# MakiseChris666/MVXNet-Makise

Measured on AMD Instinct MI355X. Metric: KITTI frames/sec (voxelize+VFE+fusion+3Dconv fwd+bwd), higher is better.
Workload: dtype f32 (bf16x6: three bf16 pieces = the f32 operand exactly, six MFMAs per product, f32 accumulate); 1 GPU; S2 ring frames (64-beam model, KITTI-like occupancy), 120000 raw pts -> 20000 pts after crop, grid 10x352x400, T=35, 4 frames/GPU/step: crop+cropToSight+lidar2Img, voxelize, fusion sampling+MLP, VFE, reindex+CML fwd+bwd, all-reduce, AdamW; convmath=bf16x6; mode=hot, frames_per_gpu=4, parallelism=dp1

## Files before the change

### mvxnet-makise_amd/csrc/activity.hip

```cpp
#include "common.h"

namespace {

constexpr int ATH = 8, ATW = 16;

__global__ void activity_sites(const void *__restrict__ src, int src_is_index, int Din, int Dout, int H, int W, int sd,
                               int pd, int mark_border, unsigned char *__restrict__ dst, int n_frames) {
    const size_t n = (size_t)n_frames * Dout * H * W;
    for (size_t e = blockIdx.x * (size_t)blockDim.x + threadIdx.x; e < n; e += (size_t)gridDim.x * blockDim.x) {
        const int x = (int)(e % W), y = (int)((e / W) % H), d = (int)(e / ((size_t)W * H));
        int on = mark_border && (y == 0 || y == H - 1 || x == 0 || x == W - 1);
        for (int kd = 0; kd < 3 && !on; ++kd) {
            const int ds = mvx_src_plane(d, Din, Dout, sd, pd, kd);
            if (ds < 0) continue;
            for (int a = -1; a <= 1 && !on; ++a) {
                const int yy = y + a;
                if (yy < 0 || yy >= H) continue;
                for (int b = -1; b <= 1; ++b) {
                    const int xx = x + b;
                    if (xx < 0 || xx >= W) continue;
                    const size_t s = ((size_t)ds * H + yy) * W + xx;
                    on |= src_is_index ? (((const int *)src)[s] >= 0) : (((const unsigned char *)src)[s] != 0);
                }
            }
        }
        dst[e] = (unsigned char)on;
    }
}


__global__ __launch_bounds__(256) void activity_sites4(const void *__restrict__ src, int src_is_index, int Din, int Dout, int H,
                                                       int W, int sd, int pd, int mark_border, unsigned char *__restrict__ dst,
                                                       int n_frames) {
    const int W4 = W >> 2;
    const size_t n = (size_t)n_frames * Dout * H * W4;
    for (size_t e = blockIdx.x * (size_t)blockDim.x + threadIdx.x; e < n; e += (size_t)gridDim.x * blockDim.x) {
        const int x = (int)(e % W4) * 4, y = (int)((e / W4) % H), d = (int)(e / ((size_t)W4 * H));
        unsigned on = 0u;
        if (mark_border) {
            if (y == 0 || y == H - 1) on = 15u;
            if (x == 0) on |= 1u;
            if (x + 4 == W) on |= 8u;
        }
        for (int kd = 0; kd < 3 && on != 15u; ++kd) {
            const int ds = mvx_src_plane(d, Din, Dout, sd, pd, kd);
            if (ds < 0) continue;
            for (int a = -1; a <= 1 && on != 15u; ++a) {
                const int yy = y + a;
                if (yy < 0 || yy >= H) continue;
                const size_t s = ((size_t)ds * H + yy) * W + x;
                unsigned m;
                if (src_is_index) {
                    const int *row = (const int *)src + s;
                    const int4 v = *(const int4 *)row;
                    m = (v.x >= 0 ? 2u : 0u) | (v.y >= 0 ? 4u : 0u) | (v.z >= 0 ? 8u : 0u) | (v.w >= 0 ? 16u : 0u);
                    if (x > 0 && row[-1] >= 0) m |= 1u;
                    if (x + 4 < W && row[4] >= 0) m |= 32u;
                } else {
                    const unsigned char *row = (const unsigned char *)src + s;
                    const unsigned v = *(const unsigned *)row;
                    m = ((v & 0xffu) ? 2u : 0u) | ((v & 0xff00u) ? 4u : 0u) | ((v & 0xff0000u) ? 8u : 0u) | ((v & 0xff000000u) ? 16u : 0u);
                    if (x > 0 && row[-1]) m |= 1u;
                    if (x + 4 < W && row[4]) m |= 32u;
                }
                on |= (m | (m >> 1) | (m >> 2)) & 15u;
            }
        }
        *(unsigned *)(dst + e * 4) = ((on & 1u) ? 1u : 0u) | ((on & 2u) ? 0x100u : 0u) | ((on & 4u) ? 0x10000u : 0u) | ((on & 8u) ? 0x1000000u : 0u);
    }
}

__global__ __launch_bounds__(256) void activity_halo_flags(const unsigned char *__restrict__ mask, int D, int H, int W,
                                                           int *__restrict__ flags, int *__restrict__ tile_flags) {
    const int tiles_x = (W + ATW - 1) / ATW;
    const int tx0 = (blockIdx.x % tiles_x) * ATW - 1, ty0 = (blockIdx.x / tiles_x) * ATH - 1;
    const int d = blockIdx.y;
    int on = 0, inner = 0;
    if (threadIdx.x < (ATH + 2) * (ATW + 2)) {
        const int hy = threadIdx.x / (ATW + 2), hx = threadIdx.x % (ATW + 2);
        const int y = ty0 + hy, x = tx0 + hx;
        if (y >= 0 && y < H && x >= 0 && x < W) on = mask[((size_t)d * H + y) * W + x];
        inner = on && hy >= 1 && hy <= ATH && hx >= 1 && hx <= ATW;
    }
    on = __syncthreads_or(on);
    inner = __syncthreads_or(inner);
    if (threadIdx.x == 0) {
        if (flags) flags[(size_t)d * gridDim.x + blockIdx.x] = on ? 1 : 0;
        if (tile_flags) tile_flags[(size_t)d * gridDim.x + blockIdx.x] = inner ? 1 : 0;
    }
}

__global__ void tile_dilate_flags(const int *__restrict__ in, const int *__restrict__ self, int Din, int Dout, int tiles_y,
                                  int tiles_x, int sd, int pd, int *__restrict__ out, int n_frames) {
    const int e = blockIdx.x * blockDim.x + threadIdx.x;
    const int nt = tiles_y * tiles_x;
    if (e >= n_frames * Dout * nt) return;
    const int d = e / nt, t = e - d * nt, ty = t / tiles_x, tx = t - ty * tiles_x;
    int on = self ? self[e] : 0;
    for (int kd = 0; kd < 3 && !on; ++kd) {
        const int ds = mvx_src_plane(d, Din, Dout, sd, pd, kd);
        if (ds < 0) continue;
        for (int a = -1; a <= 1 && !on; ++a)
            for (int b = -1; b <= 1; ++b) {
                const int yy = ty + a, xx = tx + b;
                if (yy >= 0 && yy < tiles_y && xx >= 0 && xx < tiles_x) on |= in[(size_t)ds * nt + yy * tiles_x + xx];
            }
    }
    out[e] = on ? 1 : 0;
}

__global__ __launch_bounds__(64) void conv_background(const float *__restrict__ w, const float *__restrict__ c_in, int Din,
                                                      int Dout, int Cin, int Cout, int sd, int pd,
                                                      float *__restrict__ bg_pre, float *__restrict__ bg_tap,
                                                      float *__restrict__ bg_cls) {
    const int n = blockIdx.x, d = blockIdx.y;
    double s = 0.0;
    double cls[9];
#pragma unroll
    for (int q = 0; q < 9; ++q) cls[q] = 0.0;
    for (int kd = 0; kd < 3; ++kd) {
        const int ds = mvx_src_plane(d, Din, Dout, sd, pd, kd);
        double sk = 0.0;
        if (ds >= 0)
            for (int e = threadIdx.x; e < Cin * 9; e += 64) {
                const int c = e / 9, k = e - c * 9, a = k / 3, b = k - a * 3;
                const double t = (double)w[(((size_t)n * Cin + c) * 3 + kd) * 9 + k] * (double)c_in[(size_t)ds * Cin + c];
                sk += t;
                if (bg_cls) {
#pragma unroll
                    for (int q = 0; q < 9; ++q) {
                        const int ry = q / 3, rx = q - ry * 3;
                        const bool inside = !(ry == 0 && a == 0) && !(ry == 2 && a == 2) && !(rx == 0 && b == 0) && !(rx == 2 && b == 2);
                        if (inside) cls[q] += t;
                    }
                }
            }
        s += sk;
        if (bg_tap) {
            sk = wave_sum_f64(sk);
            if (threadIdx.x == 0) bg_tap[((size_t)d * 3 + kd) * Cout + n] = (float)sk;
        }
    }
    s = wave_sum_f64(s);
    if (threadIdx.x == 0) bg_pre[(size_t)d * Cout + n] = (float)s;
    if (bg_cls) {
#pragma unroll
        for (int q = 0; q < 9; ++q) {
            const double v = wave_sum_f64(cls[q]);
            if (threadIdx.x == 0) bg_cls[((size_t)d * 9 + q) * Cout + n] = (float)v;
        }
    }
}

__global__ void bn_background(const float *__restrict__ bg_pre, const float *__restrict__ bias, const float *__restrict__ mi,
                              int D, int C, int relu, float *__restrict__ y_bg, float *__restrict__ c_out, int n_frames) {
    const int e = blockIdx.x * blockDim.x + threadIdx.x;
    if (e >= n_frames * D * C) return;
    const int c = e % C;
    mi += (size_t)(e / (D * C)) * 2 * C;
    float v = (bg_pre ? bg_pre[e] : 0.f) + (bias ? bias[c] : 0.f);
    if (relu) v = fmaxf(v, 0.f);
    if (y_bg) y_bg[e] = v;
    c_out[e] = (v - mi[c]) * mi[C + c];
}

__global__ __launch_bounds__(256) void bn_apply_tiles(const float *__restrict__ y, const float *__restrict__ mi,
                                                      const float *__restrict__ c_bg, const int *__restrict__ tile_flags,
                                                      float *__restrict__ out, int D, int H, int W, int C, int ntiles,
                                                      const int *__restrict__ read_flags) {
    const int tiles_x = (W + ATW - 1) / ATW;
    const int t = blockIdx.x, d = blockIdx.y, frame = d / D;
    if (read_flags && !read_flags[(size_t)d * ntiles + t] && !tile_flags[(size_t)d * ntiles + t]) return;
    const int c4n = C >> 2, ct = threadIdx.x % c4n, st = threadIdx.x / c4n, spb = 256 / c4n;
    const int ty0 = (t / tiles_x) * ATH, tx0 = (t % tiles_x) * ATW;
    const bool on = tile_flags[(size_t)d * ntiles + t] != 0;
    const float4 cb = *(const float4 *)(c_bg + (size_t)d * C + ct * 4);
    const float *fmi = mi + (size_t)frame * 2 * C;
    const float4 m = *(const float4 *)(fmi + ct * 4), iv = *(const float4 *)(fmi + C + ct * 4);
    for (int sidx = st; sidx < ATH * ATW; sidx += spb) {
        const int gy = ty0 + sidx / ATW, gx = tx0 + sidx % ATW;
        if (gy >= H || gx >= W) continue;
        const size_t off = (((size_t)d * H + gy) * W + gx) * C + ct * 4;
        float4 o = cb;
        if (on) {
            const float4 v = *(const float4 *)(y + off);
            o = make_float4((v.x - m.x) * iv.x, (v.y - m.y) * iv.y, (v.z - m.z) * iv.z, (v.w - m.w) * iv.w);
        }
        *(float4 *)(out + off) = o;
    }
}

__global__ void tile_read_flags(const int *__restrict__ hflag, int Din, int Dout, int ty_n, int tx_n, int sd, int pd,
                                int *__restrict__ read, int n_frames) {
    const int ntiles = ty_n * tx_n;
    const long long e = blockIdx.x * (long long)blockDim.x + threadIdx.x;
    if (e >= (long long)n_frames * Din * ntiles) return;
    const int p = (int)(e / ntiles), t = (int)(e - (long long)p * ntiles);
    const int ty = t / tx_n, tx = t - ty * tx_n;
    int r = 0;
    for (int kd = 0; kd < 3 && !r; ++kd) {
        const int d = mvx_dst_plane(p, Din, Dout, sd, pd, kd);
        if (d < 0) continue;
        for (int y = max(ty - 1, 0); y <= min(ty + 1, ty_n - 1) && !r; ++y)
            for (int x = max(tx - 1, 0); x <= min(tx + 1, tx_n - 1) && !r; ++x) {
                const int y0 = y & ~1, y1 = min(y0 + 1, ty_n - 1);
                const bool border = x == 0 || x == tx_n - 1 || y0 == 0 || y1 == ty_n - 1;
                int c = border ? 1 : 0;
                for (int k2 = 0; k2 < 3 && !c; ++k2) {
                    const int ds = mvx_src_plane(d, Din, Dout, sd, pd, k2);
                    if (ds >= 0) c = hflag[(size_t)ds * ntiles + y0 * tx_n + x] | hflag[(size_t)ds * ntiles + y1 * tx_n + x];
                }
                r |= c;
            }
    }
    read[e] = r;
}

__global__ __launch_bounds__(256) void bn_apply_tiles_bev(const float *__restrict__ y, const float *__restrict__ mi,
                                                          const float *__restrict__ c_bg, const int *__restrict__ tile_flags,
                                                          float *__restrict__ bev, int D, int H, int W, int C, int ntiles) {
    __shared__ float s_t[ATH * ATW][64 + 1];
    const int tiles_x = (W + ATW - 1) / ATW;
    const int t = blockIdx.x, d = blockIdx.y, frame = d / D, dd = d - frame * D;
    const int c4n = C >> 2, ct = threadIdx.x % c4n, st = threadIdx.x / c4n, spb = 256 / c4n;
    const int ty0 = (t / tiles_x) * ATH, tx0 = (t % tiles_x) * ATW;
    const bool on = tile_flags[(size_t)d * ntiles + t] != 0;
    const float4 cb = *(const float4 *)(c_bg + (size_t)d * C + ct * 4);
    const float *fmi = mi + (size_t)frame * 2 * C;
    const float4 m = *(const float4 *)(fmi + ct * 4), iv = *(const float4 *)(fmi + C + ct * 4);
    for (int sidx = st; sidx < ATH * ATW; sidx += spb) {
        const int gy = ty0 + sidx / ATW, gx = tx0 + sidx % ATW;
        float4 o = cb;
        if (on && gy < H && gx < W) {
            const float4 v = *(const float4 *)(y + (((size_t)d * H + gy) * W + gx) * C + ct * 4);
            o = make_float4((v.x - m.x) * iv.x, (v.y - m.y) * iv.y, (v.z - m.z) * iv.z, (v.w - m.w) * iv.w);
        }
        s_t[sidx][ct * 4 + 0] = o.x; s_t[sidx][ct * 4 + 1] = o.y; s_t[sidx][ct * 4 + 2] = o.z; s_t[sidx][ct * 4 + 3] = o.w;
    }
    __syncthreads();
    float *fb = bev + (size_t)frame * C * D * H * W;
    for (int e = threadIdx.x; e < C * ATH * (ATW / 4); e += 256) {
        const int g4 = e % (ATW / 4), c = (e / (ATW / 4)) % C, r = e / (C * (ATW / 4));
        const int gy = ty0 + r, gx = tx0 + g4 * 4;
        if (gy >= H || gx >= W) continue;
        const int s0 = r * ATW + g4 * 4;
        float *dst = fb + (((size_t)c * D + dd) * H + gy) * W + gx;
        if (gx + 3 < W && (W & 3) == 0) {
            *(float4 *)dst = make_float4(s_t[s0][c], s_t[s0 + 1][c], s_t[s0 + 2][c], s_t[s0 + 3][c]);
        } else {
            for (int j = 0; j < 4 && gx + j < W; ++j) dst[j] = s_t[s0 + j][c];
        }
    }
}

constexpr int BREP = 8;

constexpr int BNB_MAX_PLANES = 16 * MVX_MAX_FRAMES;
__global__ __launch_bounds__(1024) void bnb_tile_list(const int *__restrict__ tile_flags, int D, int H, int W, int ntiles,
                                                      int *__restrict__ list, int *__restrict__ n_act,
                                                      int *__restrict__ n_inact, unsigned *__restrict__ amax_slot) {
    __shared__ int smem[17];
    if (amax_slot && threadIdx.x == 0) *amax_slot = 0u;
    __shared__ int s_inact[BNB_MAX_PLANES];
    const int tiles_x = (W + ATW - 1) / ATW;
    if (threadIdx.x < BNB_MAX_PLANES) s_inact[threadIdx.x] = 0;
    __syncthreads();
    const int total = D * ntiles;
    int base = 0;
    for (int s0 = 0; s0 < total; s0 += 1024 * 64) {
        const int left = total - s0;
        const int per = left >= 1024 * 64 ? 64 : (left + 1023) / 1024;
        const int b0 = s0 + (int)threadIdx.x * per;
        unsigned long long bits = 0ull;
#pragma unroll 8
        for (int k = 0; k < per; ++k) {
            const int e = b0 + k;
            if (e < total) bits |= (unsigned long long)(tile_flags[e] != 0) << k;
        }
        for (int k = 0; k < per; ++k) {
            const int e = b0 + k;
            if (e < total && !((bits >> k) & 1ull)) {
                const int d = e / ntiles, t = e - d * ntiles;
                const int ty0 = (t / tiles_x) * ATH, tx0 = (t % tiles_x) * ATW;
                atomicAdd(&s_inact[d], min(ATH, H - ty0) * min(ATW, W - tx0));
            }
        }
        int tot;
        int pos = base + block_excl_scan_i32(__popcll(bits), smem, &tot);
        while (bits) {
            const int k = __ffsll((long long)bits) - 1;
            bits &= bits - 1;
            list[pos++] = b0 + k;
        }
        base += tot;
    }
    __syncthreads();
    if (threadIdx.x == 0) *n_act = base;
    if (threadIdx.x < D) n_inact[threadIdx.x] = s_inact[threadIdx.x];
}

template <int MODE>
__global__ __launch_bounds__(256) void bnb_tiles(const float *__restrict__ dyh, const float *__restrict__ y,
                                                 const float *__restrict__ mi, const float *__restrict__ c_bg,
                                                 const float *__restrict__ ab, const int *__restrict__ list,
                                                 const int *__restrict__ n_act, int D, int H, int W, int C, int ntiles,
                                                 float *__restrict__ dz, double *__restrict__ sums_all,
                                                 unsigned *__restrict__ amax_slot) {
    __shared__ float red[2][256][4];
    float mx = 0.f;
    const int tiles_x = (W + ATW - 1) / ATW;
    const int c4n = C >> 2, ct = threadIdx.x % c4n, st = threadIdx.x / c4n, spb = 256 / c4n;
    const int nact = *n_act;
    const int per = (nact + (int)gridDim.x - 1) / (int)gridDim.x;
    const int j0 = (int)blockIdx.x * per, j1 = min(nact, j0 + per);
    float4 s1 = make_float4(0.f, 0.f, 0.f, 0.f), s2 = s1;
    float4 m = s1, iv = s1, cb = s1, a = s1, b = s1;
    int cur = -1;
    auto flush = [&](int d) {
        const int frame = d / D, dl = d - frame * D;
        double *sums = sums_all + (size_t)frame * BREP * (D + 2) * C;
        __syncthreads();
        red[0][threadIdx.x][0] = s1.x; red[0][threadIdx.x][1] = s1.y; red[0][threadIdx.x][2] = s1.z; red[0][threadIdx.x][3] = s1.w;
        red[1][threadIdx.x][0] = s2.x; red[1][threadIdx.x][1] = s2.y; red[1][threadIdx.x][2] = s2.z; red[1][threadIdx.x][3] = s2.w;
        __syncthreads();
        if (st == 0) {
            const unsigned rep = blockIdx.x % BREP;
            double *base = sums + (size_t)rep * (D + 2) * C;
            for (int q4 = 0; q4 < 4; ++q4) {
                double t1 = 0.0, t2 = 0.0;
                for (int q = 0; q < spb; ++q) { t1 += (double)red[0][q * c4n + ct][q4]; t2 += (double)red[1][q * c4n + ct][q4]; }
                const int n = ct * 4 + q4;
                if (MODE == 0) {
                    atomicAdd(base + (size_t)dl * C + n, t1);
                    atomicAdd(base + (size_t)D * C + n, t2);
                } else {
                    atomicAdd(base + (size_t)(D + 1) * C + n, t1);
                }
            }
        }
        s1 = make_float4(0.f, 0.f, 0.f, 0.f); s2 = s1;
    };
    auto site = [&](const float4 g, const float4 v, size_t off) __attribute__((always_inline)) {
        const float4 yh = make_float4((v.x - m.x) * iv.x, (v.y - m.y) * iv.y, (v.z - m.z) * iv.z, (v.w - m.w) * iv.w);
        if (MODE == 0) {
            s1.x += g.x; s1.y += g.y; s1.z += g.z; s1.w += g.w;
            s2.x += g.x * (yh.x - cb.x); s2.y += g.y * (yh.y - cb.y); s2.z += g.z * (yh.z - cb.z); s2.w += g.w * (yh.w - cb.w);
        } else {
            float4 o;
            o.x = v.x > 0.f ? iv.x * (g.x - (a.x + yh.x * b.x)) : 0.f;
            o.y = v.y > 0.f ? iv.y * (g.y - (a.y + yh.y * b.y)) : 0.f;
            o.z = v.z > 0.f ? iv.z * (g.z - (a.z + yh.z * b.z)) : 0.f;
            o.w = v.w > 0.f ? iv.w * (g.w - (a.w + yh.w * b.w)) : 0.f;
            *(float4 *)(dz + off) = o;
            s1.x += o.x; s1.y += o.y; s1.z += o.z; s1.w += o.w;
            mx = fmaxf(fmaxf(mx, fmaxf(fabsf(o.x), fabsf(o.y))), fmaxf(fabsf(o.z), fabsf(o.w)));
        }
    };
    for (int j = j0; j < j1; ++j) {
        const int e = list[j], d = e / ntiles, t = e - d * ntiles;
        if (d != cur) {
            if (cur >= 0) flush(cur);
            cur = d;
            const int frame = d / D;
            const float *fmi = mi + (size_t)frame * 2 * C;
            m = *(const float4 *)(fmi + ct * 4); iv = *(const float4 *)(fmi + C + ct * 4);
            cb = *(const float4 *)(c_bg + (size_t)d * C + ct * 4);
            if (MODE == 1) { a = *(const float4 *)(ab + (size_t)frame * 2 * C + ct * 4); b = *(const float4 *)(ab + (size_t)frame * 2 * C + C + ct * 4); }
        }
        const int ty0 = (t / tiles_x) * ATH, tx0 = (t % tiles_x) * ATW;
        if (spb == ATW && ty0 + ATH <= H && tx0 + ATW <= W) {
            float4 gq[ATH], vq[ATH];
            const size_t off0 = (((size_t)d * H + ty0) * W + tx0 + st) * C + ct * 4;
#pragma unroll
            for (int r = 0; r < ATH; ++r) {
                gq[r] = *(const float4 *)(dyh + off0 + (size_t)r * W * C);
                vq[r] = *(const float4 *)(y + off0 + (size_t)r * W * C);
            }
#pragma unroll
            for (int r = 0; r < ATH; ++r) site(gq[r], vq[r], off0 + (size_t)r * W * C);
        } else {
            for (int sidx = st; sidx < ATH * ATW; sidx += spb) {
                const int gy = ty0 + sidx / ATW, gx = tx0 + sidx % ATW;
                if (gy >= H || gx >= W) continue;
                const size_t off = (((size_t)d * H + gy) * W + gx) * C + ct * 4;
                site(*(const float4 *)(dyh + off), *(const float4 *)(y + off), off);
            }
        }
    }
    if (cur >= 0) flush(cur);
    if (MODE == 1 && amax_slot) mvx_wave_amax_to(amax_slot, mx);
}

__global__ void bnb_finalize_ab(const double *__restrict__ sums, const float *__restrict__ A, const float *__restrict__ c_bg,
                                int D, int C, double count, float *__restrict__ ab) {
    const int n = blockIdx.x * blockDim.x + threadIdx.x;
    if (n >= C) return;
    const int frame = blockIdx.y;
    sums += (size_t)frame * BREP * (D + 2) * C;
    A += (size_t)frame * D * C;
    c_bg += (size_t)frame * D * C;
    ab += (size_t)frame * 2 * C;
    double q1 = 0.0;
    for (int rep = 0; rep < BREP; ++rep) q1 += sums[((size_t)rep * (D + 2) + D) * C + n];
    double sa = 0.0, sca = 0.0;
    for (int d = 0; d < D; ++d) {
        const double Ad = (double)A[(size_t)d * C + n];
        sa += Ad;
        sca += (double)c_bg[(size_t)d * C + n] * Ad;
    }
    ab[n] = (float)(sa / count);
    ab[C + n] = (float)((q1 + sca) / count);
}

__global__ void bnb_dbias(const double *__restrict__ sums, const float *__restrict__ A, const float *__restrict__ c_bg,
                          const float *__restrict__ y_bg, const float *__restrict__ mi, const float *__restrict__ ab,
                          const int *__restrict__ n_inact, int D, int C, float *__restrict__ dbias, int accumulate,
                          float *__restrict__ dz_inactive_sums, int n_frames) {
    const int n = blockIdx.x * blockDim.x + threadIdx.x;
    if (n >= C) return;
    double t = 0.0;
    for (int frame = 0; frame < n_frames; ++frame) {
        const double *fs = sums + (size_t)frame * BREP * (D + 2) * C;
        const float *fmi = mi + (size_t)frame * 2 * C, *fab = ab + (size_t)frame * 2 * C;
        double z1 = 0.0;
        for (int rep = 0; rep < BREP; ++rep) z1 += fs[((size_t)rep * (D + 2) + D + 1) * C + n];
        const double inv = (double)fmi[C + n], a = (double)fab[n], b = (double)fab[C + n];
        t += z1;
        for (int dl = 0; dl < D; ++dl) {
            const int d = frame * D + dl;
            double s = 0.0;
            if (y_bg[(size_t)d * C + n] > 0.f) {
                double p1 = 0.0;
                for (int rep = 0; rep < BREP; ++rep) p1 += fs[((size_t)rep * (D + 2) + dl) * C + n];
                s = inv * (((double)A[(size_t)d * C + n] - p1) - (double)n_inact[d] * (a + (double)c_bg[(size_t)d * C + n] * b));
            }
            if (dz_inactive_sums) dz_inactive_sums[(size_t)d * C + n] = (float)s;
            t += s;
        }
    }
    if (dbias) dbias[n] = accumulate ? dbias[n] + (float)t : (float)t;
}

}

extern "C" size_t mvx_bn_relu_backward_tiles_workspace_bytes_frames(int32_t planes, int32_t h, int32_t w, int32_t channels,
                                                                   int32_t n_frames) {
    if (planes <= 0 || planes > 16 || h <= 0 || w <= 0 || channels <= 0 || n_frames <= 0 || n_frames > MVX_MAX_FRAMES) return 0;
    const size_t ntiles = (size_t)mvx_cdiv(w, ATW) * mvx_cdiv(h, ATH);
    const size_t P = (size_t)planes * n_frames;
    return sizeof(double) * BREP * (planes + 2) * channels * n_frames + sizeof(float) * 2 * channels * n_frames +
           sizeof(int) * (P * ntiles + 16 + P);
}

extern "C" size_t mvx_bn_relu_backward_tiles_workspace_bytes(int32_t planes, int32_t h, int32_t w, int32_t channels) {
    return mvx_bn_relu_backward_tiles_workspace_bytes_frames(planes, h, w, channels, 1);
}

extern "C" int mvx_bn_relu_backward_tiles_frames(const float *dyhat, const float *y, const float *mean_inv, const float *c_bg,
                                                 const float *y_bg, const float *plane_grad_sums, const int32_t *tile_flags,
                                                 int32_t planes, int32_t h, int32_t w, int32_t channels, float *dz,
                                                 float *dbias, float *dz_inactive_sums, float *dz_amax, int32_t flags,
                                                 void *workspace, size_t workspace_bytes, int32_t n_frames, void *stream) {
    MVX_CHECK_ARG(dyhat && y && mean_inv && c_bg && y_bg && plane_grad_sums && tile_flags && dz && workspace);
    MVX_CHECK_ARG(planes > 0 && planes <= 16 && h > 0 && w > 0 && channels > 0 && channels % 4 == 0 && 256 % (channels / 4) == 0);
    MVX_CHECK_ARG(n_frames >= 1 && n_frames <= MVX_MAX_FRAMES);
    MVX_CHECK_ARG(workspace_bytes >= mvx_bn_relu_backward_tiles_workspace_bytes_frames(planes, h, w, channels, n_frames));
    hipStream_t st = (hipStream_t)stream;
    const int ntiles = (int)(mvx_cdiv(w, ATW) * mvx_cdiv(h, ATH));
    const int P = planes * n_frames;
    double *sums = (double *)workspace;
    float *ab = (float *)(sums + (size_t)BREP * (planes + 2) * channels * n_frames);
    int *list = (int *)(ab + 2 * (size_t)channels * n_frames);
    int *n_act = list + (size_t)P * ntiles, *n_inact = n_act + 16;
    hipError_t e = hipMemsetAsync(sums, 0, sizeof(double) * BREP * (planes + 2) * channels * n_frames, st);
    if (e != hipSuccess) return (int)e;
    hipLaunchKernelGGL(bnb_tile_list, dim3(1), dim3(1024), 0, st, tile_flags, P, h, w, ntiles, list, n_act, n_inact, (unsigned *)dz_amax);
    MVX_LAUNCH_CHECK();
    const double count = (double)planes * h * w;
    const unsigned grid = (unsigned)(P * ntiles > 2048 ? 2048 : P * ntiles);
    hipLaunchKernelGGL(bnb_tiles<0>, dim3(grid), dim3(256), 0, st, dyhat, y, mean_inv, c_bg, (const float *)ab, (const int *)list,
                       (const int *)n_act, planes, h, w, channels, ntiles, dz, sums, (unsigned *)nullptr);
    MVX_LAUNCH_CHECK();
    hipLaunchKernelGGL(bnb_finalize_ab, dim3(mvx_cdiv(channels, 64), n_frames), dim3(64), 0, st, (const double *)sums,
                       plane_grad_sums, c_bg, planes, channels, count, ab);
    MVX_LAUNCH_CHECK();
    hipLaunchKernelGGL(bnb_tiles<1>, dim3(grid), dim3(256), 0, st, dyhat, y, mean_inv, c_bg, (const float *)ab, (const int *)list,
                       (const int *)n_act, planes, h, w, channels, ntiles, dz, sums, (unsigned *)dz_amax);
    MVX_LAUNCH_CHECK();
    if (dbias || dz_inactive_sums) {
        hipLaunchKernelGGL(bnb_dbias, dim3(mvx_cdiv(channels, 64)), dim3(64), 0, st, (const double *)sums, plane_grad_sums, c_bg,
                           y_bg, mean_inv, (const float *)ab, (const int *)n_inact, planes, channels, dbias,
                           flags & MVX_FLAG_ACCUMULATE, dz_inactive_sums, n_frames);
        MVX_LAUNCH_CHECK();
    }
    return MVX_OK;
}

extern "C" int mvx_bn_relu_backward_tiles(const float *dyhat, const float *y, const float *mean_inv, const float *c_bg,
                                          const float *y_bg, const float *plane_grad_sums, const int32_t *tile_flags,
                                          int32_t planes, int32_t h, int32_t w, int32_t channels, float *dz, float *dbias,
                                          float *dz_inactive_sums, int32_t flags, void *workspace,
                                          size_t workspace_bytes, void *stream) {
    return mvx_bn_relu_backward_tiles_frames(dyhat, y, mean_inv, c_bg, y_bg, plane_grad_sums, tile_flags, planes, h, w, channels,
                                             dz, dbias, dz_inactive_sums, nullptr, flags, workspace, workspace_bytes, 1, stream);
}

extern "C" int mvx_activity_dilate_frames(const void *src, int32_t src_is_index, int32_t din, int32_t dout, int32_t h, int32_t w,
                                          int32_t stride_d, int32_t pad_d, int32_t mark_border, uint8_t *dst_mask,
                                          int32_t *dst_halo_flags, int32_t *dst_tile_flags, int32_t n_frames, void *stream) {
    MVX_CHECK_ARG(src && dst_mask && din > 0 && dout > 0 && h > 0 && w > 0);
    MVX_CHECK_ARG(stride_d >= 1 && stride_d <= 2 && pad_d >= 0 && pad_d <= 1);
    MVX_CHECK_ARG(dout == (din + 2 * pad_d - 3) / stride_d + 1);
    MVX_CHECK_ARG(n_frames >= 1 && n_frames <= MVX_MAX_FRAMES);
    hipStream_t st = (hipStream_t)stream;
    const size_t n = (size_t)n_frames * dout * h * w;
    if (w % 4 == 0 && ((uintptr_t)src & 15) == 0 && ((uintptr_t)dst_mask & 3) == 0)
        hipLaunchKernelGGL(activity_sites4, dim3(mvx_cdiv(n / 4, 256) > 4096 ? 4096 : mvx_cdiv(n / 4, 256)), dim3(256), 0, st, src,
                           src_is_index, din, dout, h, w, stride_d, pad_d, mark_border, dst_mask, n_frames);
    else
        hipLaunchKernelGGL(activity_sites, dim3(mvx_cdiv(n, 256) > 4096 ? 4096 : mvx_cdiv(n, 256)), dim3(256), 0, st, src,
                           src_is_index, din, dout, h, w, stride_d, pad_d, mark_border, dst_mask, n_frames);
    MVX_LAUNCH_CHECK();
    if (dst_halo_flags || dst_tile_flags) {
        hipLaunchKernelGGL(activity_halo_flags, dim3(mvx_cdiv(w, ATW) * mvx_cdiv(h, ATH), dout * n_frames), dim3(256), 0, st,
                           (const unsigned char *)dst_mask, dout * n_frames, h, w, dst_halo_flags, dst_tile_flags);
        MVX_LAUNCH_CHECK();
    }
    return MVX_OK;
}

extern "C" int mvx_activity_dilate(const void *src, int32_t src_is_index, int32_t din, int32_t dout, int32_t h, int32_t w,
                                   int32_t stride_d, int32_t pad_d, int32_t mark_border, uint8_t *dst_mask,
                                   int32_t *dst_halo_flags, int32_t *dst_tile_flags, void *stream) {
    return mvx_activity_dilate_frames(src, src_is_index, din, dout, h, w, stride_d, pad_d, mark_border, dst_mask,
                                      dst_halo_flags, dst_tile_flags, 1, stream);
}

extern "C" int mvx_tile_dilate_flags_frames(const int32_t *in_tile_flags, const int32_t *self_tile_flags, int32_t din,
                                            int32_t dout, int32_t h, int32_t w, int32_t stride_d, int32_t pad_d,
                                            int32_t *out_tile_flags, int32_t n_frames, void *stream) {
    MVX_CHECK_ARG(in_tile_flags && out_tile_flags && din > 0 && dout > 0 && h > 0 && w > 0);
    MVX_CHECK_ARG(n_frames >= 1 && n_frames <= MVX_MAX_FRAMES);
    MVX_CHECK_ARG(stride_d >= 1 && stride_d <= 2 && pad_d >= 0 && pad_d <= 1);
    MVX_CHECK_ARG(dout == (din + 2 * pad_d - 3) / stride_d + 1);
    const int ty = (int)mvx_cdiv(h, ATH), tx = (int)mvx_cdiv(w, ATW);
    hipLaunchKernelGGL(tile_dilate_flags, dim3(mvx_cdiv((long long)n_frames * dout * ty * tx, 256)), dim3(256), 0,
                       (hipStream_t)stream, in_tile_flags, self_tile_flags, din, dout, ty, tx, stride_d, pad_d, out_tile_flags,
                       n_frames);
    MVX_LAUNCH_CHECK();
    return MVX_OK;
}

extern "C" int mvx_tile_dilate_flags(const int32_t *in_tile_flags, const int32_t *self_tile_flags, int32_t din, int32_t dout,
                                     int32_t h, int32_t w, int32_t stride_d, int32_t pad_d, int32_t *out_tile_flags,
                                     void *stream) {
    return mvx_tile_dilate_flags_frames(in_tile_flags, self_tile_flags, din, dout, h, w, stride_d, pad_d, out_tile_flags, 1,
                                        stream);
}

extern "C" int mvx_conv3d_background_frames(const float *w, const float *c_in, int32_t din, int32_t dout, int32_t cin,
                                            int32_t cout, int32_t stride_d, int32_t pad_d, float *bg_pre, int32_t n_frames,
                                            void *stream) {
    MVX_CHECK_ARG(w && c_in && bg_pre && din > 0 && dout > 0 && cin > 0 && cout > 0);
    MVX_CHECK_ARG(n_frames >= 1 && n_frames <= MVX_MAX_FRAMES);
    hipLaunchKernelGGL(conv_background, dim3(cout, dout * n_frames), dim3(64), 0, (hipStream_t)stream, w, c_in, din, dout, cin,
                       cout, stride_d, pad_d, bg_pre, (float *)nullptr, (float *)nullptr);
    MVX_LAUNCH_CHECK();
    return MVX_OK;
}

extern "C" int mvx_conv3d_background_taps_frames(const float *w, const float *c_in, int32_t din, int32_t dout, int32_t cin,
                                                 int32_t cout, int32_t stride_d, int32_t pad_d, float *bg, int32_t n_frames,
                                                 void *stream) {
    MVX_CHECK_ARG(w && c_in && bg && din > 0 && dout > 0 && cin > 0 && cout > 0);
    MVX_CHECK_ARG(n_frames >= 1 && n_frames <= MVX_MAX_FRAMES);
    hipLaunchKernelGGL(conv_background, dim3(cout, dout * n_frames), dim3(64), 0, (hipStream_t)stream, w, c_in, din, dout, cin,
                       cout, stride_d, pad_d, bg, bg + (size_t)dout * n_frames * cout, bg + (size_t)4 * dout * n_frames * cout);
    MVX_LAUNCH_CHECK();
    return MVX_OK;
}

extern "C" int mvx_conv3d_background(const float *w, const float *c_in, int32_t din, int32_t dout, int32_t cin,
                                     int32_t cout, int32_t stride_d, int32_t pad_d, float *bg_pre, void *stream) {
    return mvx_conv3d_background_frames(w, c_in, din, dout, cin, cout, stride_d, pad_d, bg_pre, 1, stream);
}

extern "C" int mvx_bn_background_frames(const float *bg_pre, const float *bias, const float *mean_inv, int32_t planes,
                                        int32_t channels, int32_t flags, float *y_bg, float *c_out, int32_t n_frames,
                                        void *stream) {
    MVX_CHECK_ARG(mean_inv && c_out && planes > 0 && channels > 0 && n_frames >= 1 && n_frames <= MVX_MAX_FRAMES);
    hipLaunchKernelGGL(bn_background, dim3(mvx_cdiv((long long)n_frames * planes * channels, 256)), dim3(256), 0,
                       (hipStream_t)stream, bg_pre, bias, mean_inv, planes, channels, flags & MVX_FLAG_RELU, y_bg, c_out, n_frames);
    MVX_LAUNCH_CHECK();
    return MVX_OK;
}

extern "C" int mvx_bn_apply_tiles_frames(const float *y, const float *mean_inv, const float *c_bg, const int32_t *tile_flags,
                                         float *out, int32_t planes, int32_t h, int32_t w, int32_t channels, int32_t n_frames,
                                         void *stream) {
    MVX_CHECK_ARG(y && mean_inv && c_bg && tile_flags && out && planes > 0 && h > 0 && w > 0);
    MVX_CHECK_ARG(channels > 0 && channels % 4 == 0 && channels <= 1024 && 256 % (channels / 4) == 0);
    MVX_CHECK_ARG(n_frames >= 1 && n_frames <= MVX_MAX_FRAMES);
    const int ntiles = (int)(mvx_cdiv(w, ATW) * mvx_cdiv(h, ATH));
    hipLaunchKernelGGL(bn_apply_tiles, dim3(ntiles, planes * n_frames), dim3(256), 0, (hipStream_t)stream, y, mean_inv, c_bg,
                       (const int *)tile_flags, out, planes, h, w, channels, ntiles, (const int *)nullptr);
    MVX_LAUNCH_CHECK();
    return MVX_OK;
}

extern "C" int mvx_bn_apply_tiles_read_frames(const float *y, const float *mean_inv, const float *c_bg, const int32_t *tile_flags,
                                              const int32_t *read_flags, float *out, int32_t planes, int32_t h, int32_t w,
                                              int32_t channels, int32_t n_frames, void *stream) {
    MVX_CHECK_ARG(y && mean_inv && c_bg && tile_flags && read_flags && out && planes > 0 && h > 0 && w > 0);
    MVX_CHECK_ARG(channels > 0 && channels % 4 == 0 && channels <= 1024 && 256 % (channels / 4) == 0);
    MVX_CHECK_ARG(n_frames >= 1 && n_frames <= MVX_MAX_FRAMES);
    const int ntiles = (int)(mvx_cdiv(w, ATW) * mvx_cdiv(h, ATH));
    hipLaunchKernelGGL(bn_apply_tiles, dim3(ntiles, planes * n_frames), dim3(256), 0, (hipStream_t)stream, y, mean_inv, c_bg,
                       (const int *)tile_flags, out, planes, h, w, channels, ntiles, (const int *)read_flags);
    MVX_LAUNCH_CHECK();
    return MVX_OK;
}

extern "C" int mvx_tile_read_flags_frames(const int32_t *in_halo_flags, int32_t din, int32_t dout, int32_t h, int32_t w,
                                          int32_t stride_d, int32_t pad_d, int32_t *read_flags, int32_t n_frames, void *stream) {
    MVX_CHECK_ARG(in_halo_flags && read_flags && din > 0 && dout > 0 && h > 0 && w > 0);
    MVX_CHECK_ARG(n_frames >= 1 && n_frames <= MVX_MAX_FRAMES && stride_d >= 1 && stride_d <= 2 && pad_d >= 0 && pad_d <= 1);
    MVX_CHECK_ARG(dout == (din + 2 * pad_d - 3) / stride_d + 1);
    const int ty = (int)mvx_cdiv(h, ATH), tx = (int)mvx_cdiv(w, ATW);
    hipLaunchKernelGGL(tile_read_flags, dim3(mvx_cdiv((long long)n_frames * din * ty * tx, 256)), dim3(256), 0, (hipStream_t)stream,
                       (const int *)in_halo_flags, din, dout, ty, tx, stride_d, pad_d, (int *)read_flags, n_frames);
    MVX_LAUNCH_CHECK();
    return MVX_OK;
}

extern "C" int mvx_bn_apply_tiles_bev_frames(const float *y, const float *mean_inv, const float *c_bg, const int32_t *tile_flags,
                                             float *bev, int32_t planes, int32_t h, int32_t w, int32_t channels, int32_t n_frames,
                                             void *stream) {
    MVX_CHECK_ARG(y && mean_inv && c_bg && tile_flags && bev && planes > 0 && h > 0 && w > 0);
    MVX_CHECK_ARG(channels > 0 && channels % 4 == 0 && channels <= 64 && 256 % (channels / 4) == 0);
    MVX_CHECK_ARG(n_frames >= 1 && n_frames <= MVX_MAX_FRAMES && (((uintptr_t)bev) & 15) == 0);
    const int ntiles = (int)(mvx_cdiv(w, ATW) * mvx_cdiv(h, ATH));
    hipLaunchKernelGGL(bn_apply_tiles_bev, dim3(ntiles, planes * n_frames), dim3(256), 0, (hipStream_t)stream, y, mean_inv, c_bg,
                       (const int *)tile_flags, bev, planes, h, w, channels, ntiles);
    MVX_LAUNCH_CHECK();
    return MVX_OK;
}

extern "C" int mvx_bn_background(const float *bg_pre, const float *bias, const float *mean_inv, int32_t planes,
                                 int32_t channels, int32_t flags, float *y_bg, float *c_out, void *stream) {
    return mvx_bn_background_frames(bg_pre, bias, mean_inv, planes, channels, flags, y_bg, c_out, 1, stream);
}
```

Before: 527.7 frames/s.

## Fuse BN-ReLU backward finalize/dbias into last-block tails and pipeline tile loads

Removes the memset and the separate finalize_ab and dbias kernels. The workspace zeroing moves into the tile-list kernel, and the finalize and dbias work runs in the last-arriving block of each tile pass, detected with an atomic counter. The tile-list kernel now builds its list with wave ballots instead of a block scan, the flush reduction uses wave shuffles in double precision, and the tile loop double-buffers half-tile loads. The grid is also resized to 4x the CU count with balanced work splits. The point is fewer launches and better latency hiding, at the cost of a serial single-block tail and more complex synchronisation.

```diff
diff --git a/mvxnet-makise_amd/csrc/activity.hip b/mvxnet-makise_amd/csrc/activity.hip
--- a/mvxnet-makise_amd/csrc/activity.hip
+++ b/mvxnet-makise_amd/csrc/activity.hip
@@ -258,85 +258,203 @@
 constexpr int BNB_MAX_PLANES = 16 * MVX_MAX_FRAMES;
 __global__ __launch_bounds__(1024) void bnb_tile_list(const int *__restrict__ tile_flags, int D, int H, int W, int ntiles,
                                                       int *__restrict__ list, int *__restrict__ n_act,
-                                                      int *__restrict__ n_inact, unsigned *__restrict__ amax_slot) {
-    __shared__ int smem[17];
-    if (amax_slot && threadIdx.x == 0) *amax_slot = 0u;
+                                                      int *__restrict__ n_inact, unsigned *__restrict__ amax_slot,
+                                                      double *__restrict__ sums, int n_sums) {
+    __shared__ unsigned long long s_mask[16][64];
+    __shared__ int s_cnt[16];
     __shared__ int s_inact[BNB_MAX_PLANES];
+    for (int i = threadIdx.x; i < n_sums; i += 1024) sums[i] = 0.0;
+    if (threadIdx.x == 0) {
+        if (amax_slot) *amax_slot = 0u;
+        n_act[1] = 0; n_act[2] = 0;
+    }
     const int tiles_x = (W + ATW - 1) / ATW;
     if (threadIdx.x < BNB_MAX_PLANES) s_inact[threadIdx.x] = 0;
     __syncthreads();
     const int total = D * ntiles;
+    const int lane = threadIdx.x & 63, wave = threadIdx.x >> 6;
     int base = 0;
+    int acc = 0, acc_d = 0;
     for (int s0 = 0; s0 < total; s0 += 1024 * 64) {
-        const int left = total - s0;
-        const int per = left >= 1024 * 64 ? 64 : (left + 1023) / 1024;
-        const int b0 = s0 + (int)threadIdx.x * per;
-        unsigned long long bits = 0ull;
-#pragma unroll 8
-        for (int k = 0; k < per; ++k) {
-            const int e = b0 + k;
-            if (e < total) bits |= (unsigned long long)(tile_flags[e] != 0) << k;
-        }
-        for (int k = 0; k < per; ++k) {
-            const int e = b0 + k;
-            if (e < total && !((bits >> k) & 1ull)) {
-                const int d = e / ntiles, t = e - d * ntiles;
-                const int ty0 = (t / tiles_x) * ATH, tx0 = (t % tiles_x) * ATW;
-                atomicAdd(&s_inact[d], min(ATH, H - ty0) * min(ATW, W - tx0));
+        const int left = min(total - s0, 1024 * 64);
+        const int per = (((left + 15) >> 4) + 63) & ~63;
+        const int lo = s0 + wave * per, hi = min(s0 + left, lo + per);
+        const int trips = hi > lo ? (hi - lo + 63) >> 6 : 0;
+        int cnt = 0;
+        int d0 = lo / ntiles, r0 = lo - d0 * ntiles;
+        const bool whole = H % ATH == 0 && W % ATW == 0;
+        for (int t0 = 0; t0 < trips; t0 += 8) {
+            int fl[8];
+#pragma unroll
+            for (int k = 0; k < 8; ++k) {
+                const int e = lo + (t0 + k) * 64 + lane;
+                fl[k] = e < hi ? (tile_flags[e] != 0) : -1;
             }
-        }
-        int tot;
-        int pos = base + block_excl_scan_i32(__popcll(bits), smem, &tot);
-        while (bits) {
-            const int k = __ffsll((long long)bits) - 1;
-            bits &= bits - 1;
-            list[pos++] = b0 + k;
+#pragma unroll
+            for (int k = 0; k < 8; ++k) {
+                if (t0 + k >= trips) break;
+                const unsigned long long m = __ballot(fl[k] > 0);
+                if (lane == 0) s_mask[wave][t0 + k] = m;
+                cnt += __popcll(m);
+                if (fl[k] == 0) {
+                    int d = d0, t = r0 + lane;
+                    while (t >= ntiles) { t -= ntiles; ++d; }
+                    if (d != acc_d) {
+                        if (acc) atomicAdd(&s_inact[acc_d], acc);
+                        acc = 0; acc_d = d;
+                    }
+                    int sites = ATH * ATW;
+                    if (!whole) {
+                        const int ty0 = (t / tiles_x) * ATH, tx0 = (t % tiles_x) * ATW;
+                        sites = min(ATH, H - ty0) * min(ATW, W - tx0);
+                    }
+                    acc += sites;
+                }
+                r0 += 64;
+                while (r0 >= ntiles) { r0 -= ntiles; ++d0; }
+            }
+        }
+        if (lane == 0) s_cnt[wave] = cnt;
+        __syncthreads();
+        int pos = base, tot = 0;
+        for (int w = 0; w < 16; ++w) {
+            const int c = s_cnt[w];
+            if (w < wave) pos += c;
+            tot += c;
+        }
+        for (int t = 0; t < trips; ++t) {
+            const unsigned long long m = s_mask[wave][t];
+            if ((m >> lane) & 1ull) list[pos + __popcll(m & ((1ull << lane) - 1ull))] = lo + t * 64 + lane;
+            pos += __popcll(m);
         }
         base += tot;
-    }
+        __syncthreads();
+    }
+    if (acc) atomicAdd(&s_inact[acc_d], acc);
     __syncthreads();
     if (threadIdx.x == 0) *n_act = base;
     if (threadIdx.x < D) n_inact[threadIdx.x] = s_inact[threadIdx.x];
 }
 
+__device__ __forceinline__ bool bnb_arrived_last(unsigned *done_counter, int *s_flag) {
+    mvx_drain_vmem();
+    __syncthreads();
+    if (threadIdx.x == 0) *s_flag = (atomicAdd(done_counter, 1u) == gridDim.x - 1u);
+    __syncthreads();
+    return *s_flag != 0;
+}
+
+__device__ __forceinline__ double bnb_replica_sum(const double *p, size_t stride) {
+    double v[BREP];
+#pragma unroll
+    for (int rep = 0; rep < BREP; ++rep) v[rep] = __hip_atomic_load(p + rep * stride, __ATOMIC_RELAXED, __HIP_MEMORY_SCOPE_AGENT);
+    double t = 0.0;
+#pragma unroll
+    for (int rep = 0; rep < BREP; ++rep) t += v[rep];
+    return t;
+}
+
+__device__ __forceinline__ void bnb_finalize_ab(const double *sums_all, const float *__restrict__ A, const float *__restrict__ c_bg,
+                                                int D, int C, int n_frames, double count, float *ab) {
+    for (int e = threadIdx.x; e < C * n_frames; e += blockDim.x) {
+        const int frame = e / C, n = e - frame * C;
+        const double q1 = bnb_replica_sum(sums_all + ((size_t)frame * BREP * (D + 2) + D) * C + n, (size_t)(D + 2) * C);
+        const float *fA = A + (size_t)frame * D * C, *fc = c_bg + (size_t)frame * D * C;
+        double sa = 0.0, sca = 0.0;
+        for (int d = 0; d < D; ++d) {
+            const double Ad = (double)fA[(size_t)d * C + n];
+            sa += Ad;
+            sca += (double)fc[(size_t)d * C + n] * Ad;
+        }
+        ab[(size_t)frame * 2 * C + n] = (float)(sa / count);
+        ab[(size_t)frame * 2 * C + C + n] = (float)((q1 + sca) / count);
+    }
+}
+
+__device__ __forceinline__ void bnb_dbias(const double *sums_all, const float *__restrict__ A, const float *__restrict__ c_bg,
+                                          const float *__restrict__ y_bg, const float *__restrict__ mi, const float *ab,
+                                          const int *__restrict__ n_inact, int D, int C, int n_frames, float *__restrict__ dbias,
+                                          int accumulate, float *__restrict__ dz_inactive_sums, double *plane_terms) {
+    for (int e = threadIdx.x; e < n_frames * D * C; e += blockDim.x) {
+        const int d = e / C, n = e - d * C, frame = d / D, dl = d - frame * D;
+        double s = 0.0;
+        if (y_bg[e] > 0.f) {
+            const double *p = sums_all + ((size_t)frame * BREP * (D + 2) + dl) * C + n;
+            double p1 = 0.0;
+#pragma unroll
+            for (int rep = 0; rep < BREP; ++rep) p1 += p[(size_t)rep * (D + 2) * C];
+            const double inv = (double)mi[(size_t)frame * 2 * C + C + n];
+            const double a = (double)ab[(size_t)frame * 2 * C + n], b = (double)ab[(size_t)frame * 2 * C + C + n];
+            s = inv * (((double)A[e] - p1) - (double)n_inact[d] * (a + (double)c_bg[e] * b));
+        }
+        if (dz_inactive_sums) dz_inactive_sums[e] = (float)s;
+        plane_terms[e] = s;
+    }
+    if (!dbias) return;
+    mvx_drain_vmem();
+    __syncthreads();
+    for (int n = threadIdx.x; n < C; n += blockDim.x) {
+        double t = 0.0;
+        for (int frame = 0; frame < n_frames; ++frame) {
+            t += bnb_replica_sum(sums_all + ((size_t)frame * BREP * (D + 2) + D + 1) * C + n, (size_t)(D + 2) * C);
+            for (int dl = 0; dl < D; ++dl) t += plane_terms[((size_t)frame * D + dl) * C + n];
+        }
+        dbias[n] = accumulate ? dbias[n] + (float)t : (float)t;
+    }
+}
+
+struct BnbTail {
+    const float *A, *y_bg;
+    const int *n_inact;
+    unsigned *done_counter;
+    double *plane_terms;
+    float *dbias, *dz_inactive_sums;
+    double count;
+    int n_frames, accumulate;
+};
+
 template <int MODE>
 __global__ __launch_bounds__(256) void bnb_tiles(const float *__restrict__ dyh, const float *__restrict__ y,
-                                                 const float *__restrict__ mi, const float *__restrict__ c_bg,
-                                                 const float *__restrict__ ab, const int *__restrict__ list,
-                                                 const int *__restrict__ n_act, int D, int H, int W, int C, int ntiles,
-                                                 float *__restrict__ dz, double *__restrict__ sums_all,
-                                                 unsigned *__restrict__ amax_slot) {
-    __shared__ float red[2][256][4];
+                                                 const float *__restrict__ mi, const float *__restrict__ c_bg, float *ab,
+                                                 const int *__restrict__ list, const int *__restrict__ n_act, int D, int H,
+                                                 int W, int C, int ntiles, float *__restrict__ dz, double *sums_all,
+                                                 unsigned *__restrict__ amax_slot, BnbTail tail) {
+    constexpr int NV = MODE == 0 ? 8 : 4;
+    __shared__ double red[4][NV][64];
+    __shared__ int s_last;
     float mx = 0.f;
     const int tiles_x = (W + ATW - 1) / ATW;
     const int c4n = C >> 2, ct = threadIdx.x % c4n, st = threadIdx.x / c4n, spb = 256 / c4n;
+    const int lane = threadIdx.x & 63, wave = threadIdx.x >> 6;
     const int nact = *n_act;
-    const int per = (nact + (int)gridDim.x - 1) / (int)gridDim.x;
-    const int j0 = (int)blockIdx.x * per, j1 = min(nact, j0 + per);
+    const int per = nact / (int)gridDim.x, extra = nact % (int)gridDim.x;
+    const int j0 = (int)blockIdx.x * per + min((int)blockIdx.x, extra), j1 = j0 + per + ((int)blockIdx.x < extra ? 1 : 0);
+    const size_t row = (size_t)W * C;
     float4 s1 = make_float4(0.f, 0.f, 0.f, 0.f), s2 = s1;
     float4 m = s1, iv = s1, cb = s1, a = s1, b = s1;
     int cur = -1;
     auto flush = [&](int d) {
         const int frame = d / D, dl = d - frame * D;
-        double *sums = sums_all + (size_t)frame * BREP * (D + 2) * C;
+        double *base = sums_all + ((size_t)frame * BREP + blockIdx.x % BREP) * (D + 2) * C;
+        double v[NV];
+        v[0] = s1.x; v[1] = s1.y; v[2] = s1.z; v[3] = s1.w;
+        if (MODE == 0) { v[NV - 4] = s2.x; v[NV - 3] = s2.y; v[NV - 2] = s2.z; v[NV - 1] = s2.w; }
+        for (int off = c4n; off < 64; off <<= 1)
+#pragma unroll
+            for (int i = 0; i < NV; ++i) v[i] += __shfl_xor(v[i], off, 64);
         __syncthreads();
-        red[0][threadIdx.x][0] = s1.x; red[0][threadIdx.x][1] = s1.y; red[0][threadIdx.x][2] = s1.z; red[0][threadIdx.x][3] = s1.w;
-        red[1][threadIdx.x][0] = s2.x; red[1][threadIdx.x][1] = s2.y; red[1][threadIdx.x][2] = s2.z; red[1][threadIdx.x][3] = s2.w;
+        if (lane < c4n)
+#pragma unroll
+            for (int i = 0; i < NV; ++i) red[wave][i][lane] = v[i];
         __syncthreads();
-        if (st == 0) {
-            const unsigned rep = blockIdx.x % BREP;
-            double *base = sums + (size_t)rep * (D + 2) * C;
-            for (int q4 = 0; q4 < 4; ++q4) {
-                double t1 = 0.0, t2 = 0.0;
-                for (int q = 0; q < spb; ++q) { t1 += (double)red[0][q * c4n + ct][q4]; t2 += (double)red[1][q * c4n + ct][q4]; }
-                const int n = ct * 4 + q4;
-                if (MODE == 0) {
-                    atomicAdd(base + (size_t)dl * C + n, t1);
-                    atomicAdd(base + (size_t)D * C + n, t2);
-                } else {
-                    atomicAdd(base + (size_t)(D + 1) * C + n, t1);
-                }
-            }
+        const int wstep = c4n > 64 ? c4n >> 6 : 1;
+        for (int it = threadIdx.x; it < c4n * NV; it += 256) {
+            const int q = it % c4n, i = it / c4n;
+            double t = 0.0;
+            for (int w = q >> 6; w < 4; w += wstep) t += red[w][i][q & 63];
+            const int n = q * 4 + (i & 3);
+            if (MODE == 0) atomicAdd(base + (size_t)(i < 4 ? dl : D) * C + n, t);
+            else atomicAdd(base + (size_t)(D + 1) * C + n, t);
         }
         s1 = make_float4(0.f, 0.f, 0.f, 0.f); s2 = s1;
     };
@@ -356,89 +474,96 @@
             mx = fmaxf(fmaxf(mx, fmaxf(fabsf(o.x), fabsf(o.y))), fmaxf(fabsf(o.z), fabsf(o.w)));
         }
     };
-    for (int j = j0; j < j1; ++j) {
-        const int e = list[j], d = e / ntiles, t = e - d * ntiles;
-        if (d != cur) {
-            if (cur >= 0) flush(cur);
-            cur = d;
-            const int frame = d / D;
-            const float *fmi = mi + (size_t)frame * 2 * C;
-            m = *(const float4 *)(fmi + ct * 4); iv = *(const float4 *)(fmi + C + ct * 4);
-            cb = *(const float4 *)(c_bg + (size_t)d * C + ct * 4);
-            if (MODE == 1) { a = *(const float4 *)(ab + (size_t)frame * 2 * C + ct * 4); b = *(const float4 *)(ab + (size_t)frame * 2 * C + C + ct * 4); }
-        }
-        const int ty0 = (t / tiles_x) * ATH, tx0 = (t % tiles_x) * ATW;
-        if (spb == ATW && ty0 + ATH <= H && tx0 + ATW <= W) {
-            float4 gq[ATH], vq[ATH];
-            const size_t off0 = (((size_t)d * H + ty0) * W + tx0 + st) * C + ct * 4;
-#pragma unroll
-            for (int r = 0; r < ATH; ++r) {
-                gq[r] = *(const float4 *)(dyh + off0 + (size_t)r * W * C);
-                vq[r] = *(const float4 *)(y + off0 + (size_t)r * W * C);
-            }
-#pragma unroll
-            for (int r = 0; r < ATH; ++r) site(gq[r], vq[r], off0 + (size_t)r * W * C);
-        } else {
+    constexpr int HR = ATH / 2;
+    float4 ga[HR], va[HR], gb[HR], vb[HR];
+    auto issue = [&](float4 (&g)[HR], float4 (&v)[HR], size_t off) __attribute__((always_inline)) {
+#pragma unroll
+        for (int r = 0; r < HR; ++r) {
+            g[r] = *(const float4 *)(dyh + off + (size_t)r * row);
+            v[r] = *(const float4 *)(y + off + (size_t)r * row);
+        }
+    };
+    auto reduce = [&](const float4 (&g)[HR], const float4 (&v)[HR], size_t off) __attribute__((always_inline)) {
+#pragma unroll
+        for (int r = 0; r < HR; ++r) {
+            float4 gr = g[r], vr = v[r];
+            asm volatile("" : "+v"(gr.x), "+v"(gr.y), "+v"(gr.z), "+v"(gr.w), "+v"(vr.x), "+v"(vr.y), "+v"(vr.z), "+v"(vr.w));
+            site(gr, vr, off + (size_t)r * row);
+        }
+    };
+    auto decode = [&](int e, int &d, int &ty0, int &tx0, bool &full, size_t &off) __attribute__((always_inline)) {
+        d = e / ntiles;
+        const int t = e - d * ntiles;
+        ty0 = (t / tiles_x) * ATH; tx0 = (t % tiles_x) * ATW;
+        full = spb == ATW && ty0 + ATH <= H && tx0 + ATW <= W;
+        off = (((size_t)d * H + ty0) * W + tx0 + st) * C + ct * 4;
+    };
+    auto enter_plane = [&](int d) {
+        if (d == cur) return;
+        if (cur >= 0) flush(cur);
+        cur = d;
+        const int frame = d / D;
+        const float *fmi = mi + (size_t)frame * 2 * C;
+        m = *(const float4 *)(fmi + ct * 4); iv = *(const float4 *)(fmi + C + ct * 4);
+        cb = *(const float4 *)(c_bg + (size_t)d * C + ct * 4);
+        if (MODE == 1) { a = *(const float4 *)(ab + (size_t)frame * 2 * C + ct * 4); b = *(const float4 *)(ab + (size_t)frame * 2 * C + C + ct * 4); }
+    };
+    for (int j = j0; j < j1;) {
+        int d, ty0, tx0;
+        bool full;
+        size_t off;
+        decode(list[j], d, ty0, tx0, full, off);
+        if (!full) {
+            enter_plane(d);
             for (int sidx = st; sidx < ATH * ATW; sidx += spb) {
                 const int gy = ty0 + sidx / ATW, gx = tx0 + sidx % ATW;
                 if (gy >= H || gx >= W) continue;
-                const size_t off = (((size_t)d * H + gy) * W + gx) * C + ct * 4;
-                site(*(const float4 *)(dyh + off), *(const float4 *)(y + off), off);
+                const size_t o = (((size_t)d * H + gy) * W + gx) * C + ct * 4;
+                site(*(const float4 *)(dyh + o), *(const float4 *)(y + o), o);
             }
-        }
+            ++j;
+            continue;
+        }
+        int e1 = list[min(j + 1, j1 - 1)];
+        issue(ga, va, off);
+        bool fulln;
+        do {
+            enter_plane(d);
+            int dn, tyn, txn;
+            size_t offn;
+            decode(e1, dn, tyn, txn, fulln, offn);
+            fulln = fulln && j + 1 < j1;
+            e1 = list[min(j + 2, j1 - 1)];
+            issue(gb, vb, off + HR * row);
+            __builtin_amdgcn_sched_barrier(0);
+            reduce(ga, va, off);
+            __builtin_amdgcn_sched_barrier(0);
+            issue(ga, va, fulln ? offn : off);
+            __builtin_amdgcn_sched_barrier(0);
+            reduce(gb, vb, off + HR * row);
+            d = dn; off = offn;
+            ++j;
+        } while (fulln);
     }
     if (cur >= 0) flush(cur);
     if (MODE == 1 && amax_slot) mvx_wave_amax_to(amax_slot, mx);
-}
-
-__global__ void bnb_finalize_ab(const double *__restrict__ sums, const float *__restrict__ A, const float *__restrict__ c_bg,
-                                int D, int C, double count, float *__restrict__ ab) {
-    const int n = blockIdx.x * blockDim.x + threadIdx.x;
-    if (n >= C) return;
-    const int frame = blockIdx.y;
-    sums += (size_t)frame * BREP * (D + 2) * C;
-    A += (size_t)frame * D * C;
-    c_bg += (size_t)frame * D * C;
-    ab += (size_t)frame * 2 * C;
-    double q1 = 0.0;
-    for (int rep = 0; rep < BREP; ++rep) q1 += sums[((size_t)rep * (D + 2) + D) * C + n];
-    double sa = 0.0, sca = 0.0;
-    for (int d = 0; d < D; ++d) {
-        const double Ad = (double)A[(size_t)d * C + n];
-        sa += Ad;
-        sca += (double)c_bg[(size_t)d * C + n] * Ad;
-    }
-    ab[n] = (float)(sa / count);
-    ab[C + n] = (float)((q1 + sca) / count);
-}
-
-__global__ void bnb_dbias(const double *__restrict__ sums, const float *__restrict__ A, const float *__restrict__ c_bg,
-                          const float *__restrict__ y_bg, const float *__restrict__ mi, const float *__restrict__ ab,
-                          const int *__restrict__ n_inact, int D, int C, float *__restrict__ dbias, int accumulate,
-                          float *__restrict__ dz_inactive_sums, int n_frames) {
-    const int n = blockIdx.x * blockDim.x + threadIdx.x;
-    if (n >= C) return;
-    double t = 0.0;
-    for (int frame = 0; frame < n_frames; ++frame) {
-        const double *fs = sums + (size_t)frame * BREP * (D + 2) * C;
-        const float *fmi = mi + (size_t)frame * 2 * C, *fab = ab + (size_t)frame * 2 * C;
-        double z1 = 0.0;
-        for (int rep = 0; rep < BREP; ++rep) z1 += fs[((size_t)rep * (D + 2) + D + 1) * C + n];
-        const double inv = (double)fmi[C + n], a = (double)fab[n], b = (double)fab[C + n];
-        t += z1;
-        for (int dl = 0; dl < D; ++dl) {
-            const int d = frame * D + dl;
-            double s = 0.0;
-            if (y_bg[(size_t)d * C + n] > 0.f) {
-                double p1 = 0.0;
-                for (int rep = 0; rep < BREP; ++rep) p1 += fs[((size_t)rep * (D + 2) + dl) * C + n];
-                s = inv * (((double)A[(size_t)d * C + n] - p1) - (double)n_inact[d] * (a + (double)c_bg[(size_t)d * C + n] * b));
-            }
-            if (dz_inactive_sums) dz_inactive_sums[(size_t)d * C + n] = (float)s;
-            t += s;
-        }
-    }
-    if (dbias) dbias[n] = accumulate ? dbias[n] + (float)t : (float)t;
+    if (MODE == 1 && !tail.dbias && !tail.dz_inactive_sums) return;
+    if (!bnb_arrived_last(tail.done_counter, &s_last)) return;
+    if (MODE == 0) bnb_finalize_ab(sums_all, tail.A, c_bg, D, C, tail.n_frames, tail.count, ab);
+    else bnb_dbias(sums_all, tail.A, c_bg, tail.y_bg, mi, ab, tail.n_inact, D, C, tail.n_frames, tail.dbias, tail.accumulate,
+                   tail.dz_inactive_sums, tail.plane_terms);
+}
+
+static unsigned bnb_grid_limit() {
+    static unsigned cached = 0;
+    if (!cached) {
+        int dev = 0, cus = 0;
+        if (hipGetDevice(&dev) != hipSuccess || hipDeviceGetAttribute(&cus, hipDeviceAttributeMultiprocessorCount, dev) != hipSuccess ||
+            cus <= 0)
+            cus = 256;
+        cached = 4u * (unsigned)cus;
+    }
+    return cached;
 }
 
 }
@@ -448,7 +573,7 @@
     if (planes <= 0 || planes > 16 || h <= 0 || w <= 0 || channels <= 0 || n_frames <= 0 || n_frames > MVX_MAX_FRAMES) return 0;
     const size_t ntiles = (size_t)mvx_cdiv(w, ATW) * mvx_cdiv(h, ATH);
     const size_t P = (size_t)planes * n_frames;
-    return sizeof(double) * BREP * (planes + 2) * channels * n_frames + sizeof(float) * 2 * channels * n_frames +
+    return sizeof(double) * (BREP * (planes + 2) + planes) * channels * n_frames + sizeof(float) * 2 * channels * n_frames +
            sizeof(int) * (P * ntiles + 16 + P);
 }
 
@@ -468,31 +593,35 @@
     hipStream_t st = (hipStream_t)stream;
     const int ntiles = (int)(mvx_cdiv(w, ATW) * mvx_cdiv(h, ATH));
     const int P = planes * n_frames;
+    const int n_sums = BREP * (planes + 2) * channels * n_frames;
     double *sums = (double *)workspace;
-    float *ab = (float *)(sums + (size_t)BREP * (planes + 2) * channels * n_frames);
+    double *plane_terms = sums + n_sums;
+    float *ab = (float *)(plane_terms + (size_t)P * channels);
     int *list = (int *)(ab + 2 * (size_t)channels * n_frames);
     int *n_act = list + (size_t)P * ntiles, *n_inact = n_act + 16;
-    hipError_t e = hipMemsetAsync(sums, 0, sizeof(double) * BREP * (planes + 2) * channels * n_frames, st);
-    if (e != hipSuccess) return (int)e;
-    hipLaunchKernelGGL(bnb_tile_list, dim3(1), dim3(1024), 0, st, tile_flags, P, h, w, ntiles, list, n_act, n_inact, (unsigned *)dz_amax);
-    MVX_LAUNCH_CHECK();
-    const double count = (double)planes * h * w;
-    const unsigned grid = (unsigned)(P * ntiles > 2048 ? 2048 : P * ntiles);
-    hipLaunchKernelGGL(bnb_tiles<0>, dim3(grid), dim3(256), 0, st, dyhat, y, mean_inv, c_bg, (const float *)ab, (const int *)list,
-                       (const int *)n_act, planes, h, w, channels, ntiles, dz, sums, (unsigned *)nullptr);
-    MVX_LAUNCH_CHECK();
-    hipLaunchKernelGGL(bnb_finalize_ab, dim3(mvx_cdiv(channels, 64), n_frames), dim3(64), 0, st, (const double *)sums,
-                       plane_grad_sums, c_bg, planes, channels, count, ab);
-    MVX_LAUNCH_CHECK();
-    hipLaunchKernelGGL(bnb_tiles<1>, dim3(grid), dim3(256), 0, st, dyhat, y, mean_inv, c_bg, (const float *)ab, (const int *)list,
-                       (const int *)n_act, planes, h, w, channels, ntiles, dz, sums, (unsigned *)dz_amax);
-    MVX_LAUNCH_CHECK();
-    if (dbias || dz_inactive_sums) {
-        hipLaunchKernelGGL(bnb_dbias, dim3(mvx_cdiv(channels, 64)), dim3(64), 0, st, (const double *)sums, plane_grad_sums, c_bg,
-                           y_bg, mean_inv, (const float *)ab, (const int *)n_inact, planes, channels, dbias,
-                           flags & MVX_FLAG_ACCUMULATE, dz_inactive_sums, n_frames);
-        MVX_LAUNCH_CHECK();
-    }
+    hipLaunchKernelGGL(bnb_tile_list, dim3(1), dim3(1024), 0, st, tile_flags, P, h, w, ntiles, list, n_act, n_inact, (unsigned *)dz_amax,
+                       sums, n_sums);
+    MVX_LAUNCH_CHECK();
+    const unsigned limit = bnb_grid_limit();
+    const unsigned grid = (unsigned)P * ntiles > limit ? limit : (unsigned)P * ntiles;
+    BnbTail tail = {};
+    tail.A = plane_grad_sums;
+    tail.n_frames = n_frames;
+    tail.count = (double)planes * h * w;
+    tail.done_counter = (unsigned *)n_act + 1;
+    hipLaunchKernelGGL(bnb_tiles<0>, dim3(grid), dim3(256), 0, st, dyhat, y, mean_inv, c_bg, ab, (const int *)list, (const int *)n_act,
+                       planes, h, w, channels, ntiles, dz, sums, (unsigned *)nullptr, tail);
+    MVX_LAUNCH_CHECK();
+    tail.done_counter = (unsigned *)n_act + 2;
+    tail.y_bg = y_bg;
+    tail.n_inact = n_inact;
+    tail.plane_terms = plane_terms;
+    tail.dbias = dbias;
+    tail.accumulate = flags & MVX_FLAG_ACCUMULATE;
+    tail.dz_inactive_sums = dz_inactive_sums;
+    hipLaunchKernelGGL(bnb_tiles<1>, dim3(grid), dim3(256), 0, st, dyhat, y, mean_inv, c_bg, ab, (const int *)list, (const int *)n_act,
+                       planes, h, w, channels, ntiles, dz, sums, (unsigned *)dz_amax, tail);
+    MVX_LAUNCH_CHECK();
     return MVX_OK;
 }
 
```

After: 529.4 frames/s, median of 4. About the same (+0.3%).
